# ska-sa/katsdpsigproc

Measured on AMD Instinct MI355X. Metric: visibility samples/s (baselines x channels) through full RFI flagger, higher is better.
Workload: dtype f32 amplitude / f64 deviations

## Files before the change

katsdpsigproc_amd/csrc/ring_kernel.h:

```cpp
#pragma once
#include "fused_common.h"

#ifndef RING_STOP
#define RING_STOP 0
#endif
#define RING_THREADS 512
#define RING_STRIP 8
#define RING_NSLOT 32
#ifndef RING_G
#define RING_G 4
#endif
#ifndef RING_PRIO
#define RING_PRIO 0
#endif
#ifndef RING_STAGGER
#define RING_STAGGER 0
#endif
#define RING_SLOT_BYTES 4096
#define RING_LIST_DOUBLES 256
#define RING_XCD_GROUP 8

struct RingLayout {
    static constexpr size_t RING_BYTES = (size_t)RING_NSLOT * RING_SLOT_BYTES;
    static constexpr size_t LIST_BYTES = sizeof(double) * RING_LIST_DOUBLES * RING_STRIP;
    static constexpr size_t CTRL_BYTES = 64;
    static constexpr size_t LDS_BYTES = RING_BYTES + LIST_BYTES + CTRL_BYTES;
};

#ifdef RING_TRACE
#define RING_TRACE_STRIPS 24
#define RING_TRACE_SLOTS 16
__device__ unsigned long long ring_trace_buf[256 * 8 * RING_TRACE_STRIPS * RING_TRACE_SLOTS];
#endif

#define RING_WORK_LIST 2
#define RING_WORK_DONE 10

__device__ __forceinline__ int ring_strip_of(int x, int t)
{
    return ((t / RING_XCD_GROUP) * 8 + x) * RING_XCD_GROUP + (t % RING_XCD_GROUP);
}

__device__ __forceinline__ int ring_take(unsigned *work, int x, int n_strips, int t0)
{
    for (int k = 0; k < 8; k++) {
        const int xx = (x + k) & 7;
        const int t = t0 + (int)atomicAdd(&work[RING_WORK_LIST + xx], 1u);
        const int s = ring_strip_of(xx, t);
        if (s < n_strips) return s;
    }
    return -1;
}

__device__ __forceinline__ float ring_from_next(float v, float edge, int lane)
{
    const float r = __shfl_down(v, 1, 64);
    return lane == 63 ? edge : r;
}
__device__ __forceinline__ float ring_from_prev(float v, float edge, int lane)
{
    const float r = __shfl_up(v, 1, 64);
    return lane == 0 ? edge : r;
}

template <int WIDTH>
__global__ __launch_bounds__(RING_THREADS) void flagger_ring_kernel(const FusedParams p)
{
    constexpr int R = 64, W = WIDTH, H = WIDTH / 2;
    constexpr int G = RING_G, NSLOT = RING_NSLOT, STEPS = 64, NCHUNK = STEPS / G;
    constexpr int K = NSLOT / G;
    constexpr int PER_CHUNK = G / 2;
    static_assert(W % 2 == 1 && W <= 13 && 2 * H <= G * 3, "merging median only");
    typedef __attribute__((address_space(3))) void lds_void;
    extern __shared__ __attribute__((aligned(16))) char lds[];
    const int tid = threadIdx.x, lane = tid & 63;
    const int wave = __builtin_amdgcn_readfirstlane(tid >> 6);
    const int C = p.channels;
    double *list = (double *)(lds + RingLayout::RING_BYTES) + wave * RING_LIST_DOUBLES;
    int *ctrl = (int *)(lds + RingLayout::RING_BYTES + RingLayout::LIST_BYTES);
    const unsigned lds_base = (unsigned)(size_t)(lds_void *)lds;

    const int q = wave & 3, par = wave >> 2;
    const int rl = lane >> 2;
    const int chunk16 = (lane & 3) ^ ((rl >> 2) & 3);
    const size_t row_bytes = (size_t)p.vis_stride * 8;
    const unsigned lane_off = (unsigned)((size_t)(16 * q + rl) * 64 * row_bytes + (size_t)chunk16 * 16);
    const int pp = wave >> 1, hh = wave & 1;
    const int l16 = lane & 15;
    const unsigned rd_off = (lane >> 4) * 1024 + l16 * 64 + ((pp ^ ((l16 >> 2) & 3)) * 16) + 8 * hh;
    typedef const __attribute__((address_space(3))) char lds_cchar;
    typedef const __attribute__((address_space(3))) unsigned long long lds_cu64;
    lds_cchar *lds3 = (lds_cchar *)(lds_void *)lds;

    unsigned long long run_src = 0;
    const unsigned long long rb2 = 2 * (unsigned long long)row_bytes;
    const unsigned piece_base = __builtin_amdgcn_readfirstlane(lds_base + q * 1024);
    auto issue = [&](int slot) {
        unsigned pb = piece_base;
        asm volatile("" : "+s"(pb));
        const unsigned dst = pb + (unsigned)(slot + par) * RING_SLOT_BYTES;
        unsigned keep;
        asm volatile("s_mov_b32 %0, m0\n\ts_mov_b32 m0, %3\n\ts_nop 0\n\t"
                     "global_load_lds_dwordx4 %1, %2\n\ts_mov_b32 m0, %0"
                     : "=&s"(keep) : "v"(lane_off), "s"(run_src), "s"(dst) : "memory");
        run_src += rb2;
    };
    auto strip_base = [&](int strip) -> const char * {
        return (const char *)p.vis + (size_t)strip * (RING_STRIP * 8);
    };

    const int xcd = blockIdx.x & 7;
    const int per_list = (int)gridDim.x >> 3;
    const int t0 = p.n_static * per_list;
    auto static_strip = [&](int k) { return ring_strip_of(xcd, k * per_list + ((int)blockIdx.x >> 3)); };
    if (tid == 0) {
        int s0 = 0 < p.n_static ? static_strip(0) : ring_take(p.work, xcd, p.n_strips, t0);
        int s1 = -1;
        if (s0 >= 0) s1 = 1 < p.n_static ? static_strip(1) : ring_take(p.work, xcd, p.n_strips, t0);
        ctrl[0] = s0;
        ctrl[1] = s1;
    }
    __syncthreads();
    int cur = __builtin_amdgcn_readfirstlane(ctrl[0]), nxt = __builtin_amdgcn_readfirstlane(ctrl[1]);
    int k_strip = 0;
    auto finish = [&]() {
        if (tid == 0 && atomicAdd(&p.work[RING_WORK_DONE], 1u) == gridDim.x - 1u) {
#pragma unroll
            for (int k = RING_WORK_LIST; k <= RING_WORK_DONE; k++) p.work[k] = 0;
        }
    };
    if (cur < 0) {
        finish();
        return;
    }
#if RING_STAGGER > 0
    if ((blockIdx.x >> 3) & 1) {
#pragma unroll
        for (int i = 0; i < RING_STAGGER; i++) __builtin_amdgcn_s_sleep(127);
    }
#endif
    auto start_of = [&](int strip) -> unsigned long long {
        const unsigned long long a = (unsigned long long)strip_base(strip) + (unsigned long long)par * row_bytes;
        return ((unsigned long long)(unsigned)__builtin_amdgcn_readfirstlane((unsigned)(a >> 32)) << 32) |
               (unsigned long long)(unsigned)__builtin_amdgcn_readfirstlane((unsigned)a);
    };
    run_src = start_of(cur);
#pragma unroll
    for (int j = 0; j < NSLOT; j += 2) issue(j);
    float2 zz[2][G];
    auto read_chunk = [&](int chunk, float2 (&z)[G]) {
        unsigned ro = rd_off + ((chunk * G) % NSLOT) * RING_SLOT_BYTES;
        asm volatile("" : "+v"(ro));
#pragma unroll
        for (int g = 0; g < G; g++) {
            const unsigned long long w = *(lds_cu64 *)(lds3 + ro + g * RING_SLOT_BYTES);
            z[g] = make_float2(__uint_as_float((unsigned)w), __uint_as_float((unsigned)(w >> 32)));
        }
    };
    auto convert_chunk = [&](const float2 (&z)[G], float *a, unsigned &um) {
        static_assert(G == 4, "the pin below names four results");
        unsigned key = ~0u;
#pragma unroll
        for (int g = 0; g < G; g++) key &= ksp_abs_range_key(z[g].x, z[g].y);
#pragma unroll
        for (int g = 0; g < G; g += 2)
            ksp_abs_c64_inrange_x2(z[g].x, z[g].y, z[g + 1].x, z[g + 1].y, a[g], a[g + 1]);
        asm volatile("" : "+v"(a[0]), "+v"(a[1]), "+v"(a[2]), "+v"(a[3]));
        if (ksp_any((key & KSP_ABS_RANGE_BIT) == 0)) {
#pragma unroll
            for (int g = 0; g < G; g++) {
                a[g] = ksp_abs_c64(z[g].x, z[g].y);
                um = max(um, __float_as_uint(a[g]));
            }
        }
    };
    float amp_nxt[G];
    unsigned umax_nxt = 0;
    {
        constexpr int AH0 = (K - 1) * PER_CHUNK;
        __builtin_amdgcn_s_waitcnt(0x0070 | (AH0 & 15) | ((AH0 >> 4) << 14));
        __syncthreads();
        read_chunk(0, zz[0]);
        convert_chunk(zz[0], amp_nxt, umax_nxt);
    }
    const float nanv = __builtin_nanf("");
    const float2 *visf = (const float2 *)p.vis;

#if RING_PRIO == 1
    if (wave >= 4) __builtin_amdgcn_s_setprio(1);
#endif
    int mad_hint = -1;
    const int lane_id = lane;
#ifdef RING_TRACE
    int trace_it = 0;
#define RING_STAMP(i)                                                                              \
    do {                                                                                           \
        if (lane_id == 0 && trace_it < RING_TRACE_STRIPS && blockIdx.x < 256)                      \
            ring_trace_buf[((blockIdx.x * 8 + wave) * RING_TRACE_STRIPS + trace_it) * RING_TRACE_SLOTS + (i)] =   \
                __builtin_amdgcn_s_memtime();                                                      \
    } while (0)
#else
#define RING_STAMP(i) do { } while (0)
#endif
    for (;;) {
        int lane = lane_id;
        asm volatile("" : "+v"(lane));
        const int bl = cur * RING_STRIP + wave;
        const bool more = nxt >= 0;
        const unsigned long long start_nxt = start_of(more ? nxt : cur);
        auto fetch = [&](int c) -> float {
            const bool inside = c >= 0 && c < C;
            const int cc = inside ? c : 0;
            const float2 v = visf[(size_t)cc * p.vis_stride + bl];
            float a = ksp_abs_c64(v.x, v.y);
            return inside ? a : nanv;
        };
        RING_STAMP(0);
#ifdef RING_TRACE
        unsigned long long wait_dma = 0, wait_bar = 0;
        if (lane_id == 0 && trace_it < RING_TRACE_STRIPS && blockIdx.x < 256)
            ring_trace_buf[((blockIdx.x * 8 + wave) * RING_TRACE_STRIPS + trace_it) * RING_TRACE_SLOTS + 4] = __builtin_amdgcn_s_memrealtime();
#endif
        float amp[STEPS];
        unsigned umax = umax_nxt;
        umax_nxt = 0;
#pragma unroll
        for (int g = 0; g < G; g++) amp[g] = amp_nxt[g];
        auto load_chunk = [&](auto more_, auto c_) {
            constexpr bool MORE = decltype(more_)::value;
            constexpr int c = decltype(c_)::value;
            constexpr int AH = (K - 3) * PER_CHUNK;
#ifdef RING_TRACE
            unsigned long long w0;
            asm volatile("s_memtime %0\n\ts_waitcnt lgkmcnt(0)" : "=s"(w0));
#endif
            if constexpr (MORE || (c + K - 1) * G + G <= STEPS)
                __builtin_amdgcn_s_waitcnt(0x0070 | (AH & 15) | ((AH >> 4) << 14));
            else
                __builtin_amdgcn_s_waitcnt(0x0070);
#ifdef RING_TRACE
            unsigned long long w1;
            asm volatile("s_memtime %0\n\ts_waitcnt lgkmcnt(0)" : "=s"(w1));
#endif
#ifndef RING_NOSYNC
            __syncthreads();
#endif
#ifdef RING_TRACE
            unsigned long long w2;
            asm volatile("s_memtime %0\n\ts_waitcnt lgkmcnt(0)" : "=s"(w2));
            wait_dma += w1 - w0;
            wait_bar += w2 - w1;
#endif
            ksp_static_for<G / 2>([&](auto u_) {
                constexpr int j = c * G + 2 * decltype(u_)::value + NSLOT;
                if constexpr (j < STEPS) {
                    issue(j % NSLOT);
                } else if constexpr (MORE) {
                    if constexpr (j == STEPS) run_src = start_nxt;
                    issue(j % NSLOT);
                }
            });
            if constexpr (c == 0) read_chunk(1, zz[1]);
            if constexpr (c + 2 < NCHUNK || (MORE && c + 2 == NCHUNK)) read_chunk(c + 2, zz[c & 1]);
#if RING_PRIO == 2
            if ((c + (wave >> 2)) & 1)
                __builtin_amdgcn_s_setprio(1);
            else
                __builtin_amdgcn_s_setprio(0);
#endif
            if constexpr (c + 1 < NCHUNK)
                convert_chunk(zz[(c + 1) & 1], &amp[(c + 1) * G], umax);
            else if constexpr (MORE)
                convert_chunk(zz[(c + 1) & 1], amp_nxt, umax_nxt);
        };

        float dev[R];
        float dmax;
        unsigned ex_a = 0, ex_b = 0;
        int tiny = 0;
        auto note_exact = [&](unsigned &acc, float x, float m, float d) {
            unsigned t;
            asm("v_min_u32 %1, %2, %3\n\tv_or_b32 %1, 0x7fffff, %1\n\t"
                "v_cmp_ge_f32 vcc, %1, |%4|\n\tv_addc_co_u32 %0, vcc, %0, %0, vcc"
                : "+v"(acc), "=&v"(t)
                : "v"(__float_as_uint(x)), "v"(__float_as_uint(m)), "v"(d)
                : "vcc");
        };
        auto stream = [&](auto more_) __attribute__((always_inline)) {
#if RING_STOP == 1
            dmax = 0.f;
            ksp_static_for<NCHUNK>([&](auto c_) {
                load_chunk(more_, c_);
                constexpr int c = decltype(c_)::value;
#pragma unroll
                for (int g = 0; g < G; g++) {
                    dev[c * G + g] = amp[c * G + g];
                    dmax += amp[c * G + g];
                }
            });
#else
            MergeMedian<R, W> mm;
            mm.pinf = __builtin_inff();
            mm.ninf = -__builtin_inff();
            asm volatile("" : "+v"(mm.pinf), "+v"(mm.ninf));
            const float pinf = mm.pinf, ninf = mm.ninf;
            const bool first = lane == 0, last = lane == 63;
            dmax = ninf;
            float rh[H];
            auto X = [&](auto i_) -> float {
                constexpr int i = decltype(i_)::value;
                if constexpr (i < STEPS) {
                    if constexpr (i % G == 0) load_chunk(more_, std::integral_constant<int, i / G>{});
                    return amp[i];
                } else {
                    if constexpr (i == STEPS) {
#pragma unroll
                        for (int k = 0; k < H; k++)
                            rh[k] = ring_from_next(amp[k], (k & 1) ? ninf : pinf, lane);
                    }
                    return rh[i - STEPS];
                }
            };
            constexpr int RV = R - H;
            constexpr int STAGES = (RV + W - 1) / W;
            using MM = MergeMedian<R, W>;
            float cur_b[W];
            ksp_static_for<W>([&](auto k_) { cur_b[decltype(k_)::value] = X(k_); });
            ksp_static_for<STAGES>([&](auto m_) {
                constexpr int m = decltype(m_)::value;
                float S[MM::S_SIZE];
                S[MM::off(W - 1)] = cur_b[W - 1];
                ksp_static_for<W - 1>([&](auto u_) {
                    constexpr int t = W - 2 - decltype(u_)::value;
                    mm.template insert<W - 1 - t>(&S[MM::off(t + 1)], cur_b[t], &S[MM::off(t)]);
                });
                float P[W], nxt_b[W];
                ksp_static_for<W>([&](auto t_) {
                    constexpr int t = decltype(t_)::value;
                    constexpr int jv = m * W + t;
                    if constexpr (jv < RV) {
                        constexpr int j = jv + H;
                        if constexpr (t >= 1) {
                            nxt_b[t - 1] = X(std::integral_constant<int, (m + 1) * W + t - 1>{});
                            if constexpr (t == 1)
                                P[0] = nxt_b[0];
                            else
                                mm.template insert<t - 1>(P, nxt_b[t - 1], P);
                        }
                        const float med = mm.template rank<W - t, t, H>(&S[MM::off(t)], P);
                        const float xc = (t + H < W) ? cur_b[t + H < W ? t + H : 0] : nxt_b[t + H >= W ? t + H - W : 0];
                        float d = xc - med;
                        constexpr bool right_odd = j + H >= R && ((j + H - R + 1) & 1);
                        if constexpr (right_odd) {
                            const float lo = mm.template rank<W - t, t, H - 1>(&S[MM::off(t)], P);
                            if (last) {
                                const double dd = (double)xc - ((double)lo + (double)med) * 0.5;
                                d = (float)dd;
                                tiny += (d == 0.0f && dd != 0.0);
                            }
                        }
                        asm volatile("" : "+v"(d));
                        if constexpr (jv < 32)
                            note_exact(ex_a, xc, med, d);
                        else
                            note_exact(ex_b, xc, med, d);
                        if constexpr (jv & 1)
                            asm("v_max3_f32 %0, %0, %1, %2" : "+v"(dmax) : "v"(dev[j - 1]), "v"(d));
                        else if constexpr (jv == RV - 1)
                            dmax = mm.vmax(dmax, d);
                        dev[j] = d;
                    }
                });
                if constexpr (m + 1 < STAGES) {
                    ksp_static_for<W>([&](auto k_) {
                        constexpr int k = decltype(k_)::value;
                        constexpr int i = (m + 1) * W + k;
                        constexpr bool have = (m * W + k + 1 < RV) && (k + 1 < W);
                        if constexpr (!have) {
                            if constexpr (i < R + H)
                                nxt_b[k] = X(std::integral_constant<int, i>{});
                            else
                                nxt_b[k] = pinf;
                        }
                    });
#pragma unroll
                    for (int k = 0; k < W; k++) cur_b[k] = nxt_b[k];
                }
            });
            if constexpr (H >= 1) {
                float L[H];
#pragma unroll
                for (int k = 0; k < H; k++)
                    L[k] = ring_from_prev(amp[STEPS - H + k], ((H - k) & 1) ? pinf : ninf, lane);
                constexpr auto soff = [](int j) { return j * H - j * (j - 1) / 2; };
                float SL[H * (H + 1) / 2];
                SL[soff(H - 1)] = L[H - 1];
                ksp_static_for<H - 1>([&](auto u_) {
                    constexpr int j = H - 2 - decltype(u_)::value;
                    mm.template insert<H - 1 - j>(&SL[soff(j + 1)], L[j], &SL[soff(j)]);
                });
                float PL[2 * H];
                PL[0] = amp[0];
                ksp_static_for<H>([&](auto k_) {
                    constexpr int k = decltype(k_)::value + 1;
                    mm.template insert<k>(PL, amp[k], PL);
                });
                ksp_static_for<H>([&](auto j_) {
                    constexpr int j = decltype(j_)::value;
                    if constexpr (j >= 1) mm.template insert<j + H>(PL, amp[j + H], PL);
                    const float med = mm.template rank<H - j, j + H + 1, H>(&SL[soff(j)], PL);
                    const float xc = amp[j];
                    float d = xc - med;
                    if constexpr ((H - j) & 1) {
                        const float lo = mm.template rank<H - j, j + H + 1, H - 1>(&SL[soff(j)], PL);
                        if (first) {
                            const double dd = (double)xc - ((double)lo + (double)med) * 0.5;
                            d = (float)dd;
                            tiny += (d == 0.0f && dd != 0.0);
                        }
                    }
                    note_exact(ex_b, xc, med, d);
                    dmax = mm.vmax(dmax, d);
                    dev[j] = d;
                });
            }
#endif
        };
        if (more)
            stream(std::true_type{});
        else
            stream(std::false_type{});
        RING_STAMP(1);
#ifdef RING_TRACE
        if (lane_id == 0 && trace_it < RING_TRACE_STRIPS && blockIdx.x < 256) {
            ring_trace_buf[((blockIdx.x * 8 + wave) * RING_TRACE_STRIPS + trace_it) * RING_TRACE_SLOTS + 5] = wait_dma;
            ring_trace_buf[((blockIdx.x * 8 + wave) * RING_TRACE_STRIPS + trace_it) * RING_TRACE_SLOTS + 6] = wait_bar;
        }
#endif
        unsigned long long exact;
        {
            const unsigned ra = __builtin_bitreverse32(ex_a), rb = __builtin_bitreverse32(ex_b);
            exact = ((unsigned long long)ra << H) |
                    ((unsigned long long)(rb & ((1u << (32 - H)) - 1u)) << (H + 32)) |
                    (unsigned long long)(rb >> (32 - H));
            unsigned long long first_odd = 0, last_odd = 0;
#pragma unroll
            for (int j = 0; j < H; j++)
                if ((H - j) & 1) first_odd |= 1ull << j;
#pragma unroll
            for (int j = R - H; j < R; j++)
                if ((j + H - R + 1) & 1) last_odd |= 1ull << j;
            if (lane == 0) exact &= ~first_odd;
            if (lane == 63) exact &= ~last_odd;
        }
        if (ksp_any(umax >= 0x7f800000u)) {
            float a2[R + 2 * H];
            int c_first = lane * R - H;
            asm volatile("" : "+v"(c_first));
#pragma unroll
            for (int i = 0; i < R + 2 * H; i++) a2[i] = fetch(c_first + i);
            tiny = 0;
            median_phase_src<R, W>([&](int i) { return a2[i + H]; }, dev, dmax, &tiny);
            exact = 0;
        }
        const bool ticket = more && k_strip + 2 >= p.n_static;
        unsigned t_own = 0;
        if (tid == 0 && ticket) t_own = atomicAdd(&p.work[RING_WORK_LIST + xcd], 1u);

#if RING_STOP == 1 || RING_STOP == 2
        {
            float acc = dmax;
#pragma unroll
            for (int j = 0; j < R; j++) acc += dev[j];
            if (acc == 12345.678f && p.noise != nullptr) p.noise[bl] = acc;
        }
#else
        const double noise64 = mad_noise<R, W, RING_LIST_DOUBLES, true>(dev, lane, list, fetch, RING_STOP > 30 ? RING_STOP : 0,
#ifdef RING_TRACE
                                                                      (trace_it < RING_TRACE_STRIPS && blockIdx.x < 256)
                                                                          ? &ring_trace_buf[((blockIdx.x * 8 + wave) * RING_TRACE_STRIPS + trace_it) * RING_TRACE_SLOTS]
                                                                          : nullptr,
#else
                                                                      nullptr,
#endif
                                                                      exact, &mad_hint, tiny);
        if (lane == 0 && p.noise != nullptr) p.noise[bl] = (float)noise64;
        RING_STAMP(2);
#if RING_STOP == 3 || RING_STOP > 30
        if (noise64 == 12345.678 && p.noise != nullptr) p.noise[bl] = dmax;
#else
        const unsigned long long fl = threshold_flags<R, W>(p, dev, dmax, noise64, lane, C, fetch);
        write_flags(p, fl, lane * R, bl, C);
        RING_STAMP(3);
#endif
#endif

#ifdef RING_TRACE
        if (lane_id == 0 && trace_it < RING_TRACE_STRIPS && blockIdx.x < 256)
            ring_trace_buf[((blockIdx.x * 8 + wave) * RING_TRACE_STRIPS + trace_it) * RING_TRACE_SLOTS + 7] = (unsigned long long)cur + 1;
        trace_it++;
#endif
        if (!more) break;
        cur = nxt;
        if (!ticket) {
            nxt = static_strip(k_strip + 2);
#ifdef RING_END_SYNC
            __syncthreads();
#endif
        } else {
            if (tid == 0) {
                int take = ring_strip_of(xcd, t0 + (int)t_own);
                if (take >= p.n_strips) take = ring_take(p.work, (xcd + 1) & 7, p.n_strips, t0);
                ctrl[2] = take;
            }
            __syncthreads();
            nxt = __builtin_amdgcn_readfirstlane(ctrl[2]);
            __syncthreads();
        }
        k_strip++;
    }
    finish();
}

inline bool ring_supported(const FusedParams &p, int width)
{
    return p.channels == 4096 && width % 2 == 1 && width >= 3 && width <= 13 && !p.is_amplitude &&
           p.flags_mode == KSP_FLAGS_NONE && p.deviations == nullptr && p.work != nullptr &&
           p.baselines >= RING_STRIP && (p.vis_stride % 2) == 0 &&
           (p.threshold_kind != KSP_THRESHOLD_SUM || p.n_windows <= 4) &&
           (size_t)p.vis_stride * 8 * 4096 < 0x7fffff00ull;
}

template <int WIDTH>
inline int launch_ring(int device, hipStream_t s, const FusedParams &p_in, int n_cu, hipEvent_t ev0,
                       hipEvent_t ev1)
{
    FusedParams p = p_in;
    p.n_strips = p.baselines / RING_STRIP;
    auto kern = flagger_ring_kernel<WIDTH>;
    static std::atomic<bool> attr_set[64];
    if (device < 0 || device >= 64 || !attr_set[device].load(std::memory_order_acquire)) {
        KSP_CHECK(hipFuncSetAttribute((const void *)kern, hipFuncAttributeMaxDynamicSharedMemorySize,
                                      (int)RingLayout::LDS_BYTES));
        if (device >= 0 && device < 64) attr_set[device].store(true, std::memory_order_release);
    }
    const int grid = p.n_strips < n_cu ? p.n_strips : n_cu;
    p.n_static = 0;
    if (grid % 8 == 0 && p.n_strips / grid >= 3) {
        const int by_share = p.n_strips / grid - 2;
        const int by_range = (8 * (p.n_strips / 64)) / (grid / 8);
        p.n_static = by_share < by_range ? by_share : by_range;
    }
#ifndef RING_STATIC
    p.n_static = 0;
#endif
#ifdef RING_TRACE
    {
        void *tb = nullptr;
        KSP_CHECK(hipGetSymbolAddress(&tb, HIP_SYMBOL(ring_trace_buf)));
        KSP_CHECK(hipMemsetAsync(tb, 0, sizeof(ring_trace_buf), s));
    }
#endif
    if (ev0 != nullptr)
        hipExtLaunchKernelGGL(kern, dim3(grid), dim3(RING_THREADS), RingLayout::LDS_BYTES, s, ev0, ev1,
                              0, p);
    else
        hipLaunchKernelGGL(kern, dim3(grid), dim3(RING_THREADS), RingLayout::LDS_BYTES, s, p);
    KSP_LAUNCH_CHECK();
#ifdef RING_TRACE
    if (const char *path = getenv("KSP_RING_TRACE")) {
        KSP_CHECK(hipStreamSynchronize(s));
        const size_t n = sizeof(ring_trace_buf);
        void *host = malloc(n);
        KSP_CHECK(hipMemcpyFromSymbol(host, HIP_SYMBOL(ring_trace_buf), n));
        FILE *f = fopen(path, "wb");
        if (f != nullptr) {
            fwrite(host, 1, n, f);
            fclose(f);
        }
        free(host);
    }
#endif
    return 0;
}
```

Measured before the change: 364.1 billion.

## Fold ring DMA addressing into per-lane offsets and drop static strip schedule by default

The global_load_lds issue path now keeps a fixed scalar base per strip and advances a per-lane VGPR offset, with the slot offset folded into an immediate. This removes the 64-bit scalar add per issue and the m0 save/restore. LDS reads use absolute addresses, and the rare out-of-range branch is marked unlikely. The static strip schedule is now compiled in only under RING_STATIC, so by default every strip is taken dynamically from the work list. The ticket atomic is given a VGPR offset and its result is consumed later, so the latency can overlap with threshold work. Risks: m0 is clobbered without being restored, and the default scheduling behaviour changes.

```diff
diff --git a/katsdpsigproc_amd/csrc/ring_kernel.h b/katsdpsigproc_amd/csrc/ring_kernel.h
--- a/katsdpsigproc_amd/csrc/ring_kernel.h
+++ b/katsdpsigproc_amd/csrc/ring_kernel.h
@@ -87,36 +87,48 @@
     const unsigned lane_off = (unsigned)((size_t)(16 * q + rl) * 64 * row_bytes + (size_t)chunk16 * 16);
     const int pp = wave >> 1, hh = wave & 1;
     const int l16 = lane & 15;
-    const unsigned rd_off = (lane >> 4) * 1024 + l16 * 64 + ((pp ^ ((l16 >> 2) & 3)) * 16) + 8 * hh;
-    typedef const __attribute__((address_space(3))) char lds_cchar;
+    const unsigned rd_off = lds_base + (lane >> 4) * 1024 + l16 * 64 + ((pp ^ ((l16 >> 2) & 3)) * 16) + 8 * hh;
     typedef const __attribute__((address_space(3))) unsigned long long lds_cu64;
-    lds_cchar *lds3 = (lds_cchar *)(lds_void *)lds;
-
-    unsigned long long run_src = 0;
-    const unsigned long long rb2 = 2 * (unsigned long long)row_bytes;
-    const unsigned piece_base = __builtin_amdgcn_readfirstlane(lds_base + q * 1024);
-    auto issue = [&](int slot) {
-        unsigned pb = piece_base;
-        asm volatile("" : "+s"(pb));
-        const unsigned dst = pb + (unsigned)(slot + par) * RING_SLOT_BYTES;
-        unsigned keep;
-        asm volatile("s_mov_b32 %0, m0\n\ts_mov_b32 m0, %3\n\ts_nop 0\n\t"
-                     "global_load_lds_dwordx4 %1, %2\n\ts_mov_b32 m0, %0"
-                     : "=&s"(keep) : "v"(lane_off), "s"(run_src), "s"(dst) : "memory");
-        run_src += rb2;
+
+    unsigned long long run_base = 0;
+    const unsigned rb2 = __builtin_amdgcn_readfirstlane((unsigned)(2 * row_bytes));
+    unsigned run_off = lane_off - rb2;
+    const unsigned piece_base =
+        __builtin_amdgcn_readfirstlane(lds_base + q * 1024 + par * RING_SLOT_BYTES);
+    auto issue = [&](auto slot_) {
+        constexpr unsigned slot_off = decltype(slot_)::value * RING_SLOT_BYTES;
+        unsigned &off = run_off;
+        const unsigned long long src = run_base;
+        const unsigned dst = piece_base, step = rb2;
+        unsigned long long base;
+        asm volatile("s_mov_b64 %1, %2\n\ts_add_u32 m0, %3, %4\n\tv_add_u32 %0, %5, %0\n\t"
+                     "global_load_lds_dwordx4 %0, %1"
+                     : "+v"(off), "=&s"(base)
+                     : "s"(src), "s"(dst), "i"(slot_off), "s"(step)
+                     : "memory", "scc");
+    };
+    auto next_strip = [&](unsigned long long start) {
+        run_base = start;
+        run_off -= 32 * rb2;
     };
     auto strip_base = [&](int strip) -> const char * {
         return (const char *)p.vis + (size_t)strip * (RING_STRIP * 8);
     };
 
     const int xcd = blockIdx.x & 7;
+#ifdef RING_STATIC
+    const int n_static = p.n_static;
     const int per_list = (int)gridDim.x >> 3;
-    const int t0 = p.n_static * per_list;
+    const int t0 = n_static * per_list;
     auto static_strip = [&](int k) { return ring_strip_of(xcd, k * per_list + ((int)blockIdx.x >> 3)); };
+#else
+    constexpr int n_static = 0, t0 = 0;
+    auto static_strip = [&](int) { return -1; };
+#endif
     if (tid == 0) {
-        int s0 = 0 < p.n_static ? static_strip(0) : ring_take(p.work, xcd, p.n_strips, t0);
+        int s0 = 0 < n_static ? static_strip(0) : ring_take(p.work, xcd, p.n_strips, t0);
         int s1 = -1;
-        if (s0 >= 0) s1 = 1 < p.n_static ? static_strip(1) : ring_take(p.work, xcd, p.n_strips, t0);
+        if (s0 >= 0) s1 = 1 < n_static ? static_strip(1) : ring_take(p.work, xcd, p.n_strips, t0);
         ctrl[0] = s0;
         ctrl[1] = s1;
     }
@@ -144,16 +156,15 @@
         return ((unsigned long long)(unsigned)__builtin_amdgcn_readfirstlane((unsigned)(a >> 32)) << 32) |
                (unsigned long long)(unsigned)__builtin_amdgcn_readfirstlane((unsigned)a);
     };
-    run_src = start_of(cur);
-#pragma unroll
-    for (int j = 0; j < NSLOT; j += 2) issue(j);
+    run_base = start_of(cur);
+    ksp_static_for<NSLOT / 2>([&](auto u_) { issue(std::integral_constant<int, 2 * decltype(u_)::value>{}); });
     float2 zz[2][G];
     auto read_chunk = [&](int chunk, float2 (&z)[G]) {
         unsigned ro = rd_off + ((chunk * G) % NSLOT) * RING_SLOT_BYTES;
         asm volatile("" : "+v"(ro));
 #pragma unroll
         for (int g = 0; g < G; g++) {
-            const unsigned long long w = *(lds_cu64 *)(lds3 + ro + g * RING_SLOT_BYTES);
+            const unsigned long long w = *(lds_cu64 *)(size_t)(ro + g * RING_SLOT_BYTES);
             z[g] = make_float2(__uint_as_float((unsigned)w), __uint_as_float((unsigned)(w >> 32)));
         }
     };
@@ -166,7 +177,7 @@
         for (int g = 0; g < G; g += 2)
             ksp_abs_c64_inrange_x2(z[g].x, z[g].y, z[g + 1].x, z[g + 1].y, a[g], a[g + 1]);
         asm volatile("" : "+v"(a[0]), "+v"(a[1]), "+v"(a[2]), "+v"(a[3]));
-        if (ksp_any((key & KSP_ABS_RANGE_BIT) == 0)) {
+        if (__builtin_expect(ksp_any((key & KSP_ABS_RANGE_BIT) == 0), 0)) {
 #pragma unroll
             for (int g = 0; g < G; g++) {
                 a[g] = ksp_abs_c64(z[g].x, z[g].y);
@@ -254,10 +265,10 @@
             ksp_static_for<G / 2>([&](auto u_) {
                 constexpr int j = c * G + 2 * decltype(u_)::value + NSLOT;
                 if constexpr (j < STEPS) {
-                    issue(j % NSLOT);
+                    issue(std::integral_constant<int, j % NSLOT>{});
                 } else if constexpr (MORE) {
-                    if constexpr (j == STEPS) run_src = start_nxt;
-                    issue(j % NSLOT);
+                    if constexpr (j == STEPS) next_strip(start_nxt);
+                    issue(std::integral_constant<int, j % NSLOT>{});
                 }
             });
             if constexpr (c == 0) read_chunk(1, zz[1]);
@@ -463,9 +474,14 @@
             median_phase_src<R, W>([&](int i) { return a2[i + H]; }, dev, dmax, &tiny);
             exact = 0;
         }
-        const bool ticket = more && k_strip + 2 >= p.n_static;
+        const bool ticket = more && k_strip + 2 >= n_static;
         unsigned t_own = 0;
-        if (tid == 0 && ticket) t_own = atomicAdd(&p.work[RING_WORK_LIST + xcd], 1u);
+        if (tid == 0 && ticket) {
+            unsigned counter = (RING_WORK_LIST + xcd) * (unsigned)sizeof(unsigned);
+            asm volatile("" : "+v"(counter));
+            t_own = atomicAdd((unsigned *)((char *)p.work + counter), 1u);
+        }
+        auto land_ticket = [&]() { asm volatile("" : "+v"(t_own)); };
 
 #if RING_STOP == 1 || RING_STOP == 2
         {
@@ -490,6 +506,7 @@
         if (noise64 == 12345.678 && p.noise != nullptr) p.noise[bl] = dmax;
 #else
         const unsigned long long fl = threshold_flags<R, W>(p, dev, dmax, noise64, lane, C, fetch);
+        land_ticket();
         write_flags(p, fl, lane * R, bl, C);
         RING_STAMP(3);
 #endif
@@ -508,6 +525,7 @@
             __syncthreads();
 #endif
         } else {
+            land_ticket();
             if (tid == 0) {
                 int take = ring_strip_of(xcd, t0 + (int)t_own);
                 if (take >= p.n_strips) take = ring_take(p.work, (xcd + 1) & 7, p.n_strips, t0);
```

After: 366.1 billion, median of 5. About the same (+0.6%).
